# georgegrosu1/torch-admm-deconv

Hardware: AMD Instinct MI355X
Metric: ADMM iterations/sec, batch-64 1024x1024x3, 50 iters; rel-L2 vs CPU ref (higher is better)
Workload: dtype f32

## Files before the change

torch-admm-deconv_amd/csrc/admm_capi.hip:

```cpp
#include <hip/hip_runtime.h>

#include <cstdlib>
#include <cstring>
#include <mutex>
#include <string>
#include <type_traits>
#include <vector>

#include "gcol_mm.hpp"
#include "knobs.hpp"
#include "mixed_capi.hpp"
#include "odd_capi.hpp"
#include "admm_tv.h"

using namespace admm;

namespace {

thread_local std::string g_err;

int fail(int code, const std::string& msg) {
    g_err = msg;
    return code;
}
// ... 221 lines not shown
int launch_check(const char* what) {
    hipError_t e = hipGetLastError();
    if (e != hipSuccess) return fail(ADMM_TV_EHIP, std::string(what) + ": " + hipGetErrorString(e));
    return 0;
}

int hip_code(hipError_t e, const char* what) {
    return e == hipSuccess ? 0 : fail(ADMM_TV_EHIP, std::string(what) + ": " + hipGetErrorString(e));
}

int check_workspace(const void* ws, size_t have, size_t need) {
    if (!ws || have < need || (reinterpret_cast<uintptr_t>(ws) % kAlign) != 0)
        return fail(ADMM_TV_EWORKSPACE, "workspace too small or not 256-byte aligned");
    return 0;
}

template <class T>
int bwd_scalars(double* part, int K, long long nstrips, long long spm, long long soff, const double* tpart, int ntp,
                int G, int g, const T* lam, const T* rho, T* glam, T* grho, hipStream_t s) {
    if (K < 1) return fail(ADMM_TV_EINVAL, "bwd_scalars: no iterations");
    hipLaunchKernelGGL(k_bwd_iter_sums, dim3((unsigned)K), dim3(256), 0, s, part, nstrips, spm, soff, tpart, ntp, G, g);
    if (int e = launch_check("k_bwd_iter_sums")) return e;
    hipLaunchKernelGGL(k_bwd_scalars<T>, dim3(1), dim3(256), 0, s, (const double*)part, K, nstrips, 1LL, soff,
                       (const double*)nullptr, ntp, G, g, lam, rho, glam, grho);
    return launch_check("k_bwd_scalars");
}

template <int N> struct RowOps {
    using G = RowKernelGeom<N>;
    static unsigned blocks(long long items) { return (unsigned)((items + G::SG - 1) / G::SG); }

    static int r2c(const float* img, cf* spec, const cf* twW, long long rows, hipStream_t s, bool pl = false) {
        if (pl)
            hipLaunchKernelGGL((k_row_r2c<N, true>), dim3(blocks(rows)), dim3(G::NT), G::lds_bytes(), s, img, spec, twW, rows);
        else
            hipLaunchKernelGGL((k_row_r2c<N, false>), dim3(blocks(rows)), dim3(G::NT), G::lds_bytes(), s, img, spec, twW, rows);
        return launch_check("k_row_r2c");
    }
    static int c2r(const cf* spec, float* img, const cf* twW, long long rows, hipStream_t s, bool pl = false) {
        if (pl)
            hipLaunchKernelGGL((k_row_c2r<N, true>), dim3(blocks(rows)), dim3(G::NT), G::lds_bytes(), s, spec, img, twW, rows);
        else
            hipLaunchKernelGGL((k_row_c2r<N, false>), dim3(blocks(rows)), dim3(G::NT), G::lds_bytes(), s, spec, img, twW, rows);
        return launch_check("k_row_c2r");
    }
    static int pair(const float* img, float* out, long long rows, hipStream_t s) {
        hipLaunchKernelGGL(k_row_pair<N>, dim3(blocks(rows)), dim3(G::NT), 0, s, img, out, rows);
        return launch_check("k_row_pair");
    }
    template <bool ISO, bool FIRST, bool HIST, bool PL> static void pa(const PassAArgs& a, unsigned nb, hipStream_t s) {
        hipLaunchKernelGGL((k_pass_a<N, ISO, FIRST, HIST, PL>), dim3(nb), dim3(G::NT), G::lds_bytes(), s, a);
    }
    static constexpr bool kCoop = N == 512;
    template <bool FIRST, bool PL> static void pa_coop(const PassAArgs& a, unsigned nb, hipStream_t s) {
        if constexpr (kCoop)
            hipLaunchKernelGGL((k_pass_a<N, false, FIRST, false, PL, true>), dim3(nb), dim3(G::NT), passa_coop_lds<N>(), s, a);
    }
    static int pass_a(const PassAArgs& a, bool iso, bool first, bool hist, hipStream_t s, bool pl = false,
                      bool coop = false) {
        const unsigned nb = blocks(a.nstrips);
        const int sel = (iso ? 4 : 0) | (first ? 2 : 0) | (hist ? 1 : 0);
        if (kCoop && coop && !iso && !hist && !a.rev && a.R >= 2 && a.nstrips % G::SG == 0 &&
            (a.H / a.R) % G::SG == 0) {
            static_assert(!kCoop || passa_coop_lds<N>() <= 53 * 1024, "three blocks of the row pass per CU");
            if (first) pl ? pa_coop<true, true>(a, nb, s) : pa_coop<true, false>(a, nb, s);
            else pl ? pa_coop<false, true>(a, nb, s) : pa_coop<false, false>(a, nb, s);
            return launch_check("k_pass_a");
        }
        if (pl && !hist) {
            switch (sel) {
                case 0: pa<false, false, false, true>(a, nb, s); break;
                case 2: pa<false, true, false, true>(a, nb, s); break;
                case 4: pa<true, false, false, true>(a, nb, s); break;
                default: pa<true, true, false, true>(a, nb, s); break;
            }
            return launch_check("k_pass_a");
        }
        switch (sel) {
            case 0: pa<false, false, false, false>(a, nb, s); break;
            case 1: pa<false, false, true, false>(a, nb, s); break;
            case 2: pa<false, true, false, false>(a, nb, s); break;
            case 3: pa<false, true, true, false>(a, nb, s); break;
            case 4: pa<true, false, false, false>(a, nb, s); break;
            case 5: pa<true, false, true, false>(a, nb, s); break;
            case 6: pa<true, true, false, false>(a, nb, s); break;
            default: pa<true, true, true, false>(a, nb, s); break;
        }
        return launch_check("k_pass_a");
    }
    static int iso_norm(const IsoArgs& a, bool first, bool hist, hipStream_t s, bool pl = false) {
        const unsigned nb = blocks(a.nitems);
        if (first && pl)
            hipLaunchKernelGGL((k_iso_norm<N, true, false, true>), dim3(nb), dim3(G::NT), G::lds_bytes(), s, a);
        else if (first)
            hipLaunchKernelGGL((k_iso_norm<N, true, false, false>), dim3(nb), dim3(G::NT), G::lds_bytes(), s, a);
        else if (hist)
            hipLaunchKernelGGL((k_iso_norm<N, false, true, false>), dim3(nb), dim3(G::NT), G::lds_bytes(), s, a);
        else if (pl)
            hipLaunchKernelGGL((k_iso_norm<N, false, false, true>), dim3(nb), dim3(G::NT), G::lds_bytes(), s, a);
        else
            hipLaunchKernelGGL((k_iso_norm<N, false, false, false>), dim3(nb), dim3(G::NT), G::lds_bytes(), s, a);
        return launch_check("k_iso_norm");
    }
    template <bool ISO, bool LASTK, bool FIRSTK> static void bpa(const BwdArgs& a, unsigned nb, hipStream_t s) {
        using BG = BwdGeom<N>;
        hipLaunchKernelGGL((k_bwd_pass_a<N, ISO, LASTK, FIRSTK>), dim3(nb), dim3(BG::NT), BG::lds_bytes(), s, a);
    }
    static int bwd_pass_a(const BwdArgs& a, bool iso, bool lastk, bool firstk, hipStream_t s) {
        const unsigned nb = (unsigned)((a.nstrips + BwdGeom<N>::SG - 1) / BwdGeom<N>::SG);
        const int sel = (iso ? 4 : 0) | (lastk ? 2 : 0) | (firstk ? 1 : 0);
        switch (sel) {
            case 0: bpa<false, false, false>(a, nb, s); break;
            case 1: bpa<false, false, true>(a, nb, s); break;
            case 2: bpa<false, true, false>(a, nb, s); break;
            case 3: bpa<false, true, true>(a, nb, s); break;
            case 4: bpa<true, false, false>(a, nb, s); break;
            case 5: bpa<true, false, true>(a, nb, s); break;
            case 6: bpa<true, true, false>(a, nb, s); break;
            default: bpa<true, true, true>(a, nb, s); break;
// ... 170 lines not shown
    hipLaunchKernelGGL(k_tables<C>, dim3((std::max(H, W) + nt - 1) / nt), dim3(nt), 0, s, at<C>(ws, Lo.twW),
                       at<C>(ws, Lo.twH), at<double2>(ws, Lo.twHd), H, W);
    if (int e = launch_check("k_tables")) return e;
    if (Lo.gen && !std::is_same<T, double>::value) {
        for (int dim = 0; dim < 2; ++dim) {
            const GPlan pl = make_plan(dim == 0 ? W : H);
            if (pl.ntab == 0) continue;
            hipLaunchKernelGGL(k_blue_tables, dim3((3 * 1024 * 64 + nt - 1) / nt), dim3(nt), 0, s,
                               at<cf>(ws, dim == 0 ? Lo.twW : Lo.twH), pl);
            if (int e = launch_check("k_blue_tables")) return e;
        }
    }
    if (k > 0) {
        const int n = k * (N + 1);
        hipLaunchKernelGGL(k_psf_rows<T>, dim3((n + nt - 1) / nt), dim3(nt), 0, s, kern, at<double2>(ws, Lo.G), k, N, W);
        if (int e = launch_check("k_psf_rows")) return e;
    }
    const int n = (N + 1) * H;
    if (rho) {
        for (int g = 0; g < ngroups_of(d); ++g) {
            hipLaunchKernelGGL(k_spectra<T>, dim3((n + nt - 1) / nt), dim3(nt), 0, s, at<double2>(ws, Lo.G),
                               at<double2>(ws, Lo.twHd), rho + g, at<T>(ws, Lo.fcT) + (size_t)g * n, at<C>(ws, Lo.mT),
                               k, H, N, W, Lo.sigma ? at<double2>(ws, Lo.sigma) : nullptr,
                               (std::is_same<T, double>::value ? 1.0 / ((double)H * W) : spectra_scale(H, W)));
            if (int e = launch_check("k_spectra")) return e;
            if constexpr (std::is_same<T, float>::value) if (!Lo.gen) {
                float* fc = at<float>(ws, Lo.fcT) + (size_t)g * n;
                hipLaunchKernelGGL(k_fc_pack, dim3((n + nt - 1) / nt), dim3(nt), 0, s, fc,
                                   fc + (size_t)ngroups_of(d) * n, H, N, col_e(H));
                if (int e = launch_check("k_fc_pack")) return e;
            }
            if constexpr (std::is_same<T, float>::value) if (Lo.mixed) {
                if (int e = hip_code(admm_mixed::fc_mixed(at<float>(ws, Lo.fcT) + (size_t)g * n,
                                                          at<float>(ws, Lo.fcM) + (size_t)g * (2 * N + 1) * H, H, N, s),
                                     "k_fc_mixed"))
                    return e;
            }
            if constexpr (std::is_same<T, float>::value) if (Lo.gen && Lo.mm.ok && ngroups_of(d) == 1) {
                float* fc = at<float>(ws, Lo.fcT);
                hipLaunchKernelGGL(k_fc_transpose, dim3(std::min(4096, (n + nt - 1) / nt)), dim3(nt), 0, s, fc, fc + n, H,
                                   N + 1);
                if (int e = launch_check("k_fc_transpose")) return e;
            }
        }
        if constexpr (std::is_same<T, float>::value) if (Lo.mixed && k > 0) {
            if (int e = hip_code(admm_mixed::mt_mixed(at<cf>(ws, Lo.mT), at<cf>(ws, Lo.mM), H, N, s), "k_mt_mixed")) return e;
        }
    }
    return 0;
}

int pow2_floor(int v);

int strip_rows(int H, int N, long long rows, bool aniso_fwd = false) {
    int R = env_int("ADMM_PASSA_R", 0);
    if (R > 0) R = pow2_floor(std::max(2, std::min(R, H)));
    if (R <= 0) {
        const int L = std::min(64, N / (N >= 1024 ? 16 : N >= 64 ? 8 : N >= 16 ? 4 : 2));
        long long want = 3LL * 1024 * 64 / L;
        R = 8;
        if (aniso_fwd && N == 256) {
            R = 16;
            want /= 2;
        }
        while (R > 2 && rows / R < want) R /= 2;
    }
    if (R > H) R = H;
    return R;
}

struct DeviceGuard {
    int prev = -1, dev = -1;
    hipError_t err = hipSuccess;
    explicit DeviceGuard(hipStream_t s) {
        err = hipGetDevice(&prev);
        if (err != hipSuccess) return;
        dev = prev;
        if (s) {
            hipDevice_t d = 0;
            err = hipStreamGetDevice(s, &d);
            if (err != hipSuccess) return;
            dev = (int)d;
        }
        if (dev != prev) err = hipSetDevice(dev);
    }
    ~DeviceGuard() {
        if (prev >= 0 && dev != prev) (void)hipSetDevice(prev);
    }
    int check() const {
        return err == hipSuccess ? 0 : fail(ADMM_TV_EHIP, std::string("device of the stream: ") + hipGetErrorString(err));
    }
};

constexpr int kMaxAux = 3;
struct AuxEntry {
    hipStream_t caller = nullptr, aux[kMaxAux] = {};
};
constexpr int kAuxDev = 64, kAuxPerDev = 32;
struct AuxPool {
    std::mutex mu;
    AuxEntry e[kAuxDev][kAuxPerDev];
    int used[kAuxDev] = {}, next[kAuxDev] = {};
} g_aux;

hipStream_t aux_stream(hipStream_t s, int dev, int k = 0) {
    if (dev < 0 || dev >= kAuxDev || k < 0 || k >= kMaxAux) return nullptr;
    std::lock_guard<std::mutex> lk(g_aux.mu);
    AuxEntry* row = g_aux.e[dev];
    AuxEntry* slot = nullptr;
    for (int i = 0; i < g_aux.used[dev] && !slot; ++i)
        if (row[i].caller == s) slot = &row[i];
    if (!slot) {
        if (g_aux.used[dev] < kAuxPerDev) {
            slot = &row[g_aux.used[dev]++];
        } else {
            slot = &row[g_aux.next[dev]];
            g_aux.next[dev] = (g_aux.next[dev] + 1) % kAuxPerDev;
// ... 755 lines not shown
}

long long mixed_slots(int N) {
    static std::mutex mu;
    static std::vector<std::pair<std::pair<int, int>, long long>> cache;
    int dev = 0;
    if (hipGetDevice(&dev) != hipSuccess) return 512;
    std::lock_guard<std::mutex> lk(mu);
    for (const auto& c : cache)
        if (c.first.first == dev && c.first.second == N) return c.second;
    long long slots = 0;
    int cus = 0;
    if (hipDeviceGetAttribute(&cus, hipDeviceAttributeMultiprocessorCount, dev) == hipSuccess)
        slots = (long long)cus * std::max(1, admm_mixed::pass_a_blocks_per_cu(N));
    if (slots <= 0) return 512;
    cache.push_back({{dev, N}, slots});
    return slots;
}
int strip_rows_mixed(int H, long long rows, int N, long long slots = 0) {
    if (const int e = env_int("ADMM_MIXED_R", 0); e > 0 && H % e == 0) return e;
    const int sg = 256 / std::max(1, admm_mixed::row_lanes(N));
    if (slots <= 0) slots = mixed_slots(N);
    int best = 1;
    double best_t = 1e300;
    for (int R = 1; R <= 32 && R <= H; ++R) {
        if (H % R) continue;
        const long long strips = rows / R;
        const long long blocks = (strips + sg - 1) / sg;
        const double t = (double)((blocks + slots - 1) / slots) * (R + 1);
        if (t < best_t - 1e-9 || (t < best_t + 1e-9 && R > best)) {
            best_t = t;
            best = R;
        }
    }
    return best;
}

struct FusedOps {
    const admm_tv_desc& d;
    const Layout& Lo;
    void* const ws;
    const int H, N;
    cf *const twW, *const twH;
    FusedOps(const admm_tv_desc& d_, const Layout& L, void* w)
        : d(d_), Lo(L), ws(w), H((int)d_.H), N((int)d_.W / 2), twW(at<cf>(w, L.twW)), twH(at<cf>(w, L.twH)) {}
};

struct Pow2Ops : FusedOps {
    static constexpr bool kPsfGrad = true;
    float* const fcT;
    cf* const mT;
    const bool coop;
    const int rev;
    Pow2Ops(const admm_tv_desc& d_, const Layout& L, void* w)
        : FusedOps(d_, L, w), fcT(at<float>(w, L.fcT)), mT(at<cf>(w, L.mT)),
          coop(env_int("ADMM_PASSA_COOP", 1) != 0), rev(env_int("ADMM_PASSA_REV", 0)) {}
    int modules_per_pass(int G) const { return G; }
    bool lane_paired(bool train) const { return !train && env_int("ADMM_PL", (d.iso || d.W < 1024) ? 1 : 0) != 0; }
    int strip(long long rows, bool aniso_fwd) const { return strip_rows(H, N, rows, aniso_fwd); }
    int r2c(const float* img, cf* spec, long long rows, hipStream_t s, bool pl = false) const {
        return with_row(N, [&](auto ops) { return decltype(ops)::r2c(img, spec, twW, rows, s, pl); });
    }
    int c2r(const cf* spec, float* img, long long rows, hipStream_t s) const {
        return with_row(N, [&](auto ops) { return decltype(ops)::c2r(spec, img, twW, rows, s); });
    }
    int col(const cf* in, cf* out, long long np, long long ppm, int , hipStream_t s) const {
        return pass_b_oop(H, in, out, fcT, mT, twH, N, (int)np, 0, s, (int)ppm);
    }
    int xspec(const cf* U, const cf* V, cf* part, long long P, int ppg, bool , hipStream_t s) const {
        return ::xspec(H, U, V, part, twH, N, (int)P, ppg, s);
    }
    int iso_norm(const IsoArgs& a, bool first, bool hist, hipStream_t s, bool pl) const {
        return with_row(N, [&](auto ops) { return decltype(ops)::iso_norm(a, first, hist, s, pl); });
    }
    int pass_a(const PassAArgs& a, bool iso, bool first, bool hist, hipStream_t s, bool pl) const {
        return with_row(N, [&](auto ops) { return decltype(ops)::pass_a(a, iso, first, hist, s, pl, coop); });
    }
    int bwd_iso_q(const BwdIsoArgs& a, bool lastk, hipStream_t s) const {
        return with_row(N, [&](auto ops) { return decltype(ops)::bwd_iso_q(a, lastk, s); });
    }
    int bwd_pass_a(const BwdArgs& a, bool iso, bool lastk, bool firstk, hipStream_t s) const {
        return with_row(N, [&](auto ops) { return decltype(ops)::bwd_pass_a(a, iso, lastk, firstk, s); });
    }
    int make_b(const float* xin, float* bb, cf* spec, bool pl, hipStream_t s) const {
        if (d.kh > 0) return psf_transpose_into(d, Lo, ws, xin, bb, spec, 1, s, pl);
        return with_row(N, [&](auto ops) { return decltype(ops)::pair(xin, bb, d.B * d.C * H, s); });
    }
    int apply_ht_t(const float* bbar, float* gxin, cf* spec, hipStream_t s) const {
        return psf_transpose_into(d, Lo, ws, bbar, gxin, spec, 2, s);
    }
};

struct MixedOps : FusedOps {
    static constexpr bool kPsfGrad = true;
    const float* const fcM;
    static constexpr int rev = 0;
    MixedOps(const admm_tv_desc& d_, const Layout& L, void* w) : FusedOps(d_, L, w), fcM(at<float>(w, L.fcM)) {}
    int modules_per_pass(int) const { return 1; }
    bool lane_paired(bool) const { return false; }
    int strip(long long rows, bool) const { return strip_rows_mixed(H, rows, N); }
    int r2c(const float* img, cf* spec, long long rows, hipStream_t s, bool = false) const {
        return hip_code(admm_mixed::r2c(N, img, spec, twW, rows, s), "k_row_r2c_m");
    }
    int c2r(const cf* spec, float* img, long long rows, hipStream_t s) const {
        return hip_code(admm_mixed::c2r(N, spec, img, twW, rows, s), "k_row_c2r_m");
    }
    int col(const cf* in, cf* out, long long np, long long, int g0, hipStream_t s) const {
        return hip_code(admm_mixed::pass_b(H, in, out, fcM + (size_t)g0 * (2 * N + 1) * H, twH, N, np, s), "k_pass_b_m");
    }
    int xspec(const cf* U, const cf* V, cf* part, long long P, int ppg, bool weighted, hipStream_t s) const {
        return hip_code(admm_mixed::xspec(H, U, V, part, twH, N, P, ppg, weighted ? 0.25f : 1.f, s), "k_xspec_m");
    }
    int iso_norm(const IsoArgs& a, bool first, bool hist, hipStream_t s, bool) const {
        return hip_code(admm_mixed::iso_norm(N, a, first, hist, s), "k_iso_norm_m");
    }
    int pass_a(const PassAArgs& a, bool iso, bool first, bool hist, hipStream_t s, bool) const {
        return hip_code(admm_mixed::pass_a(N, a, iso, first, hist, s), "k_pass_a_m");
    }
    int bwd_iso_q(const BwdIsoArgs& a, bool lastk, hipStream_t s) const {
        return hip_code(admm_mixed::bwd_iso_q(N, a, lastk, s), "k_bwd_iso_q_m");
    }
    int bwd_pass_a(const BwdArgs& a, bool iso, bool lastk, bool firstk, hipStream_t s) const {
        return hip_code(admm_mixed::bwd_pass_a(N, a, iso, lastk, firstk, s), "k_bwd_pass_a_m");
    }
    int make_b(const float* xin, float* bb, cf* spec, bool, hipStream_t s) const {
        const long long P = d.B * d.C;
        if (env_int("ADMM_MIXED_BGEN", 0)) return gapply<float>(xin, bb, spec, Lo, ws, d, 1, s);
        if (int e = r2c(xin, spec, P * H, s)) return e;
        if (int e = hip_code(admm_mixed::pass_b_cm(H, spec, at<cf>(ws, Lo.mM), twH, N, P, s), "k_pass_b_m<cm>")) return e;
// ... 683 lines not shown
```

torch-admm-deconv_amd/csrc/admm_kernels.hpp:

```cpp
#pragma once
#include "fft_core.hpp"

namespace admm {

template <int N, class Cfg = RowCfg<N>> struct RowXf {
    static constexpr int E = Cfg::E;
    static constexpr int L = N / E;
    static constexpr int W = 2 * N;
    static_assert(L <= 64, "row transforms keep one row inside one wave");

    __device__ __forceinline__ static void partner(const cf (&v)[E], cf (&p)[E], int t) {
        const int src = (L - t) & (L - 1);
#pragma unroll
        for (int j = 0; j < E; ++j) {
            float a = __shfl(v[E - 1 - j].x, src, L);
            float b = __shfl(v[E - 1 - j].y, src, L);
            p[j] = (t == 0) ? v[(E - j) & (E - 1)] : mkc(a, b);
        }
    }

    __device__ __forceinline__ static void c2r(cf (&v)[E], const RowBuf& buf, const cf* __restrict__ tw, int t) {
        cf p[E];
        partner(v, p, t);
#pragma unroll
        for (int j = 0; j < E; ++j) {
            const int k = t + L * j;
            cf z;
            if (j == 0 && t == 0) {
                z = mkc(v[0].x + v[0].y, v[0].x - v[0].y);
            } else {
                cf pc = cconj(p[j]);
                cf e = cadd(v[j], pc);
                cf o = cmulc(csub(v[j], pc), tw[k]);
                z = mkc(e.x - o.y, e.y + o.x);
            }
            v[j] = z;
        }
        fft_e<N, L, E, +1, 0, 2>(v, buf, tw, t, typename Cfg::S{});
    }

    __device__ __forceinline__ static void r2c(cf (&v)[E], const RowBuf& buf, const cf* __restrict__ tw, int t) {
        fft_e<N, L, E, -1, 0, 2>(v, buf, tw, t, typename Cfg::S{});
        cf p[E];
        partner(v, p, t);
#pragma unroll
        for (int j = 0; j < E; ++j) {
            const int k = t + L * j;
            cf z;
            if (j == 0 && t == 0) {
                z = mkc(2.f * (v[0].x + v[0].y), 2.f * (v[0].x - v[0].y));
            } else {
                cf pc = cconj(p[j]);
                cf s = cadd(v[j], pc);
                cf d = cmul(csub(v[j], pc), tw[k]);
                z = mkc(s.x + d.y, s.y - d.x);
            }
            v[j] = z;
        }
    }
};

__device__ __forceinline__ float soft(float a, float tau) {
    float m = fabsf(a) - tau;
    m = (m < 0.f) ? 0.f : m;
    return copysignf(m, a);
}
__device__ __forceinline__ float block_factor(float sumsq, float tau) {
    float n = sqrtf(sumsq + 1e-15f);
    float f = 1.f - tau / (n + 1e-15f);
    return f < 0.f ? 0.f : f;
}
template <class T> __device__ __forceinline__ constexpr T eps15() {
    if constexpr (std::is_same<T, float>::value) return 1e-15f;
    else return 1e-15;
}
__device__ __forceinline__ double soft(double a, double tau) {
    double m = fabs(a) - tau;
    m = (m < 0.0) ? 0.0 : m;
    return copysign(m, a);
}
__device__ __forceinline__ double block_factor(double sumsq, double tau) {
    double n = sqrt(sumsq + 1e-15);
    double f = 1.0 - tau / (n + 1e-15);
    return f < 0.0 ? 0.0 : f;
}

template <class C = cf>
__global__ void k_tables(C* __restrict__ twW, C* __restrict__ twH, double2* __restrict__ twHd, int H, int W) {
    using T = re_t<C>;
    const int i = blockIdx.x * blockDim.x + threadIdx.x;
    if (i < W) {
        double s, c;
        sincospi(2.0 * i / W, &s, &c);
        twW[i] = mkx<T>((T)c, (T)-s);
    }
// ... 42 lines not shown
    if (sigma_out) sigma_out[i] = make_double2(sr, si);
    const double rho = (double)rho_p[0];
    const double sx = sinpi((double)kx / W), sy = sinpi((double)ky / H);
    const double lap = 4.0 * sx * sx + 4.0 * sy * sy;
    fcT[i] = (T)(scale / (sr * sr + si * si + rho * lap));
    if (k > 0) {
        const int c = k / 2;
        const long long ph = (long long)c * ky * W + (long long)c * kx * H;
        const long long HW = (long long)H * W;
        double s, co;
        sincospi(2.0 * (double)(ph % HW) / (double)HW, &s, &co);
        mT[i] = mkx<T>((T)((sr * co - si * s) * scale), (T)((sr * s + si * co) * scale));
    }
}

template <int N> struct RowKernelGeom {
    static constexpr int E = RowCfg<N>::E, L = N / E, W = 2 * N;
    static constexpr int NT = 256, SG = NT / L;
    static constexpr size_t lds_bytes() { return sizeof(cf) * (W + SG * RowBuf::slots(N)); }
};

__device__ __forceinline__ void load_tw(cf* dst, const cf* __restrict__ src, int n) {
    for (int i = threadIdx.x; i < n; i += blockDim.x) dst[i] = src[i];
}

typedef float f4v __attribute__((ext_vector_type(4)));
template <int E, int L, bool PL, bool NT> __device__ __forceinline__ void ld_row(const cf* row, int t, cf (&v)[E]) {
    if constexpr (PL) {
        static_assert(E % 2 == 0, "lane-paired rows need an even number of values per lane");
        const f4v* r4 = reinterpret_cast<const f4v*>(row);
#pragma unroll
        for (int j = 0; j < E / 2; ++j) {
            const f4v q = NT ? __builtin_nontemporal_load(&r4[t + L * j]) : r4[t + L * j];
            v[2 * j] = mkc(q.x, q.y);
            v[2 * j + 1] = mkc(q.z, q.w);
        }
    } else {
#pragma unroll
        for (int j = 0; j < E; ++j) v[j] = ld_pol<NT>(&row[t + L * j]);
    }
}
template <int E, int L, bool PL, bool NT> __device__ __forceinline__ void st_row(cf* row, int t, const cf (&v)[E]) {
    if constexpr (PL) {
        f4v* r4 = reinterpret_cast<f4v*>(row);
#pragma unroll
        for (int j = 0; j < E / 2; ++j) {
            const f4v q = {v[2 * j].x, v[2 * j].y, v[2 * j + 1].x, v[2 * j + 1].y};
            if constexpr (NT) __builtin_nontemporal_store(q, &r4[t + L * j]);
            else r4[t + L * j] = q;
        }
    } else {
#pragma unroll
        for (int j = 0; j < E; ++j) st_pol<NT>(&row[t + L * j], v[j]);
    }
}

template <int N, bool PL>
__global__ void __launch_bounds__(256) k_row_r2c(const float* __restrict__ img, cf* __restrict__ spec,
                                                 const cf* __restrict__ twW_g, long long rows) {
    using G = RowKernelGeom<N>;
    constexpr int E = G::E, L = G::L;
    extern __shared__ __attribute__((aligned(16))) unsigned char smem[];
    cf* tw = reinterpret_cast<cf*>(smem);
    load_tw(tw, twW_g, G::W);
    __syncthreads();
    const int sgl = threadIdx.x / L, t = threadIdx.x % L;
    const long long row = (long long)blockIdx.x * G::SG + sgl;
    if (row >= rows) return;
    RowBuf buf{tw + G::W + sgl * RowBuf::slots(N)};
    const cf* src = reinterpret_cast<const cf*>(img + row * G::W);
    cf v[E];
    ld_row<E, L, PL, false>(src, t, v);
    RowXf<N>::r2c(v, buf, tw, t);
    cf* dst = spec + row * N;
#pragma unroll
    for (int j = 0; j < E; ++j) dst[t + L * j] = v[j];
}

template <int N, bool PL>
__global__ void __launch_bounds__(256) k_row_c2r(const cf* __restrict__ spec, float* __restrict__ img,
                                                 const cf* __restrict__ twW_g, long long rows) {
    using G = RowKernelGeom<N>;
    constexpr int E = G::E, L = G::L;
    extern __shared__ __attribute__((aligned(16))) unsigned char smem[];
    cf* tw = reinterpret_cast<cf*>(smem);
    load_tw(tw, twW_g, G::W);
    __syncthreads();
    const int sgl = threadIdx.x / L, t = threadIdx.x % L;
    const long long row = (long long)blockIdx.x * G::SG + sgl;
    if (row >= rows) return;
    RowBuf buf{tw + G::W + sgl * RowBuf::slots(N)};
    const cf* src = spec + row * N;
    cf v[E];
#pragma unroll
    for (int j = 0; j < E; ++j) v[j] = src[t + L * j];
    RowXf<N>::c2r(v, buf, tw, t);
    cf* dst = reinterpret_cast<cf*>(img + row * G::W);
    st_row<E, L, PL, false>(dst, t, v);
}

template <int N>
__global__ void __launch_bounds__(256) k_row_pair(const float* __restrict__ img, float* __restrict__ out, long long rows) {
    using G = RowKernelGeom<N>;
    constexpr int E = G::E, L = G::L;
    const int sgl = threadIdx.x / L, t = threadIdx.x % L;
    const long long row = (long long)blockIdx.x * G::SG + sgl;
// ... 250 lines not shown
    fft<H, L, +1, 1, 1>(v1, buf, tw, t);
#pragma unroll
    for (int j = 0; j < E; ++j) bstore_f4(ro, voff, j * sstep, make_float4(v0[j].x, v0[j].y, v1[j].x, v1[j].y));
}

struct PassAArgs {
    const cf* sin;
    cf* sout;
    const float* b;
    const float* uxi;
    const float* uyi;
    float* uxo;
    float* uyo;
    const float* nsq;
    const float* nsq_prev;
    const float* lam;
    const float* rho;
    const cf* twW;
    int H;
    int R;
    long long nstrips;
    long long ppm;
    int rev = 0;
};

#ifndef PASSA_MINW_SMALL
#define PASSA_MINW_SMALL 3
#endif
#define PASSA_MINW(n) ((n) >= 1024 ? 1 : PASSA_MINW_SMALL)

template <bool ISO, class T> __device__ __forceinline__ T shrink_z(T a, T tau, T nsum) {
    if constexpr (ISO) return block_factor(nsum, tau) * a;
    else return soft(a, tau);
}

template <bool ISO, bool FIRST, bool HIST>
__device__ __forceinline__ cf prev_u(const cf* __restrict__ src, const cf* __restrict__ nsp, size_t idx, float tau) {
    if constexpr (FIRST) {
        return mkc(0.f, 0.f);
    } else {
        const cf v = lda<16>(&src[idx]);
        if constexpr (HIST) {
            const cf n = ISO ? nsp[idx] : mkc(0.f, 0.f);
            return mkc(v.x - shrink_z<ISO>(v.x, tau, n.x), v.y - shrink_z<ISO>(v.y, tau, n.y));
        } else {
            return v;
        }
    }
}

template <int N> constexpr size_t passa_coop_lds() {
    return RowKernelGeom<N>::lds_bytes() + sizeof(cf) * (RowKernelGeom<N>::SG - 1) * N;
}
template <int N, bool ISO, bool FIRST, bool HIST, bool PL, bool COOP = false>
__global__ void __launch_bounds__(256, PASSA_MINW(N)) k_pass_a(PassAArgs a) {
    static_assert(!(PL && HIST), "the training history keeps the pixel-order layout");
    using G = RowKernelGeom<N>;
    constexpr int E = G::E, L = G::L, W = G::W, SG = G::SG;
    static_assert(!COOP || (L == 64 && SG % 2 == 0 && !HIST && !ISO), "cooperative strips: whole waves in pairs, aniso inference");
    constexpr bool kSpecNT = (ADMM_NT & 2) != 0 || ((ADMM_NT & 32) != 0 && N >= 512);
    extern __shared__ __attribute__((aligned(16))) unsigned char smem[];
    cf* tw = reinterpret_cast<cf*>(smem);
    load_tw(tw, a.twW, W);
    __syncthreads();
    const int sgl = COOP ? __builtin_amdgcn_readfirstlane(threadIdx.x / L) : threadIdx.x / L, t = threadIdx.x % L;
#ifndef ADMM_PASSA_REMAP
#define ADMM_PASSA_REMAP -1
#endif
    constexpr bool kRemap = ADMM_PASSA_REMAP < 0 ? N <= 256 : ADMM_PASSA_REMAP != 0;
    const unsigned blk = kRemap ? xcd_remap(blockIdx.x, gridDim.x) : blockIdx.x;
    long long strip = (long long)blk * G::SG + sgl;
    if constexpr (!COOP) {
        if (strip >= a.nstrips) return;
        if (a.rev) strip = a.nstrips - 1 - strip;
    }
    const int H = a.H, R = a.R;
    const int spp = H / R;
    const long long p = strip / spp;
    const int i0 = (int)(strip % spp) * R;
    RowBuf buf{tw + W + sgl * RowBuf::slots(N)};
    const int mod = (int)(p / a.ppm);
    const float rho = a.rho[mod];
    const float tau = a.lam[mod] / rho;

    const cf* sp = a.sin + (size_t)p * H * N;
    cf* so = a.sout + (size_t)p * H * N;
    const size_t poff = (size_t)p * H * W;
    const cf* bimg = reinterpret_cast<const cf*>(a.b + (size_t)(p - (long long)mod * a.ppm) * H * W);
    const cf* uxi = reinterpret_cast<const cf*>(a.uxi + poff);
    const cf* uyi = reinterpret_cast<const cf*>(a.uyi + poff);
    const bool ust = HIST || a.uxo != nullptr;
    cf* uxo = ust ? reinterpret_cast<cf*>(a.uxo + poff) : nullptr;
    cf* uyo = ust ? reinterpret_cast<cf*>(a.uyo + poff) : nullptr;
    const size_t moff = (size_t)mod * 2 * H * W;
    const cf* nsx = reinterpret_cast<const cf*>(a.nsq + moff);
    const cf* nsy = reinterpret_cast<const cf*>(a.nsq + moff + (size_t)H * W);
    const cf* npx = reinterpret_cast<const cf*>(a.nsq_prev + moff);
    const cf* npy = reinterpret_cast<const cf*>(a.nsq_prev + moff + (size_t)H * W);

    auto xrow = [&](int g, cf (&x)[E]) __attribute__((always_inline)) {
#pragma unroll
        for (int j = 0; j < E; ++j) x[j] = ld_pol<kSpecNT>(&sp[(size_t)g * N + t + L * j]);
        RowXf<N>::c2r(x, buf, tw, t);
    };
    auto ydir = [&](int g, const cf (&xg)[E], const cf (&xup)[E], bool store, cf (&wyc)[E]) __attribute__((always_inline)) {
        const size_t ro = (size_t)g * N;
        {
            cf uy[E], fy[E];
            if constexpr (PL) {
                if constexpr (FIRST) {
#pragma unroll
                    for (int j = 0; j < E; ++j) uy[j] = mkc(0.f, 0.f);
// ... 79 lines not shown
                const float n0 = a0 - z0, n1 = a1 - z1;
                ux[j] = HIST ? mkc(a0, a1) : mkc(n0, n1);
                wxp[j] = mkc(z0 - n0, z1 - n1);
            }
            if (ust) {
                if constexpr (PL) {
                    st_row<E, L, true, (ADMM_NT & 1) != 0>(uxo + ro, t, ux);
                } else {
#pragma unroll
                    for (int j = 0; j < E; ++j) sta(&uxo[ro + t + L * j], ux[j]);
                }
            }
        }
    };

    cf xprev[E], xcur[E], wxp[E], wyp[E], wyc[E];
    auto pick = [](bool c, cf p, cf q) __attribute__((always_inline)) { return mkc(c ? p.x : q.x, c ? p.y : q.y); };
    auto ystep = [&](bool up, int gy, bool store) __attribute__((always_inline)) {
        cf xg[E], xup[E];
#pragma unroll
        for (int j = 0; j < E; ++j) {
            xg[j] = pick(up, xprev[j], xcur[j]);
            xup[j] = pick(up, xcur[j], xprev[j]);
        }
        ydir(gy, xg, xup, store, wyc);
    };
    auto fstep = [&](bool up, int gf) __attribute__((always_inline)) {
        cf wa[E], wb[E];
#pragma unroll
        for (int j = 0; j < E; ++j) {
            wa[j] = pick(up, wyc[j], wyp[j]);
            wb[j] = pick(up, wyp[j], wyc[j]);
        }
        finish(gf, wxp, wa, wb);
    };
    auto shift = [&]() __attribute__((always_inline)) {
#pragma unroll
        for (int j = 0; j < E; ++j) {
            wyp[j] = wyc[j];
            xprev[j] = xcur[j];
        }
    };
    auto step = [&](bool up, int g, bool ystore, bool fin, bool xd) __attribute__((always_inline)) {
        xrow(g, xcur);
        const int gn = up ? (g + 1) & (H - 1) : g;
        ystep(up, gn, ystore);
        if (fin) fstep(up, up ? gn : (g - 1 + H) & (H - 1));
        if (xd) xdir(g, xcur, wxp);
        shift();
    };
    if constexpr (!COOP) {
        xrow((i0 - 1 + H) & (H - 1), xprev);
        for (int rr = 0; rr <= R; ++rr) step(false, (i0 + rr) & (H - 1), rr < R, rr >= 1, rr < R);
    } else {
        cf* mbox = tw + W + SG * RowBuf::slots(N);
        const bool up = (sgl & 1) != 0, top = sgl == 0, bot = sgl == SG - 1;
        cf* mbs = mbox + (size_t)min(max(up ? sgl : sgl - 1, 0), SG - 2) * N;
        cf* mbe = mbox + (size_t)(up ? sgl - 1 : sgl) * N;
        auto put = [&](cf* mb, const cf (&v)[E]) __attribute__((always_inline)) {
#pragma unroll
            for (int j = 0; j < E; ++j) mb[t + L * j] = v[j];
        };
        auto get = [&](const cf* mb, cf (&v)[E]) __attribute__((always_inline)) {
#pragma unroll
            for (int j = 0; j < E; ++j) v[j] = mb[t + L * j];
        };
        const int gs = up ? i0 + R - 1 : i0;
        if (top || bot) xrow((top ? i0 - 1 + H : i0 + R) & (H - 1), xprev);
        xrow(gs, xcur);
        if (up && !bot) put(mbs, xcur);
        lds_barrier();
        if (!up && !top) get(mbs, xprev);
        if (!up || bot) ystep(up, up ? (i0 + R) & (H - 1) : gs, !up);
        if (!up && !top) put(mbs, wyc);
        lds_barrier();
        if (up && !bot) get(mbs, wyc);
        xdir(gs, xcur, wxp);
        shift();
        for (int rr = 1; rr < R; ++rr) step(up, up ? i0 + R - 1 - rr : i0 + rr, true, true, true);
        if (!up) put(mbe, xprev);
        lds_barrier();
        if (up) {
            get(mbe, xcur);
            ystep(true, i0, true);
            put(mbe, wyc);
        }
        lds_barrier();
        if (!up) get(mbe, wyc);
        fstep(up, up ? i0 : i0 + R - 1);
    }
}

struct IsoArgs {
    const cf* sin;
    const float* uxi;
    const float* uyi;
    const float* nsq_prev;
    const float* lam;
    const float* rho;
    float* partial;
    const cf* twW;
    int P, H, ppg;
    long long nitems;
    long long ppm;
};

// ... 96 lines not shown
```

torch-admm-deconv_amd/csrc/fft_core.hpp:

```cpp
#pragma once
#include <hip/hip_runtime.h>
#include <type_traits>

namespace admm {

typedef float2 cf;

__device__ __forceinline__ cf mkc(float r, float i) { cf z; z.x = r; z.y = i; return z; }
__device__ __forceinline__ cf cadd(cf a, cf b) { return mkc(a.x + b.x, a.y + b.y); }
__device__ __forceinline__ cf csub(cf a, cf b) { return mkc(a.x - b.x, a.y - b.y); }
__device__ __forceinline__ cf cmul(cf a, cf b) {
    return mkc(fmaf(a.x, b.x, -(a.y * b.y)), fmaf(a.x, b.y, a.y * b.x));
}
__device__ __forceinline__ cf cmulc(cf a, cf b) {
    return mkc(fmaf(a.x, b.x, a.y * b.y), fmaf(a.y, b.x, -(a.x * b.y)));
}
__device__ __forceinline__ cf cconj(cf a) { return mkc(a.x, -a.y); }
__device__ __forceinline__ cf cscale(cf a, float s) { return mkc(a.x * s, a.y * s); }
template <int DIR> __device__ __forceinline__ cf mul_i(cf a) {
    return DIR < 0 ? mkc(a.y, -a.x) : mkc(-a.y, a.x);
}

typedef double2 cd;
__device__ __forceinline__ cd mkcd(double r, double i) { cd z; z.x = r; z.y = i; return z; }
// ... 126 lines not shown
    __device__ __forceinline__ static void combine(cf (&v)[E], cf (&e)[R / 2], cf (&o)[R / 2]) {
        if constexpr (K < R / 2) {
            cf t = tw_mul<R, DIR, K>(o[K]);
            v[OFF + K * STRIDE] = cadd(e[K], t);
            v[OFF + (K + R / 2) * STRIDE] = csub(e[K], t);
            combine<K + 1, STRIDE, OFF>(v, e, o);
        }
    }
    template <int STRIDE, int OFF, int E> __device__ __forceinline__ static void run(cf (&v)[E]) {
        cf e[R / 2], o[R / 2];
#pragma unroll
        for (int i = 0; i < R / 2; ++i) {
            e[i] = v[OFF + (2 * i) * STRIDE];
            o[i] = v[OFF + (2 * i + 1) * STRIDE];
        }
        DFT<R / 2, DIR>::template run<1, 0>(e);
        DFT<R / 2, DIR>::template run<1, 0>(o);
        combine<0, STRIDE, OFF>(v, e, o);
    }
};

template <int... Rs> struct Sched {};

template <int N> struct RowCfg;
template <> struct RowCfg<8> { static constexpr int E = 2; using S = Sched<2, 2, 2>; };
template <> struct RowCfg<16> { static constexpr int E = 4; using S = Sched<4, 4>; };
template <> struct RowCfg<32> { static constexpr int E = 4; using S = Sched<4, 4, 2>; };
template <> struct RowCfg<64> { static constexpr int E = 8; using S = Sched<8, 8>; };
template <> struct RowCfg<128> { static constexpr int E = 8; using S = Sched<8, 8, 2>; };
template <> struct RowCfg<256> { static constexpr int E = 8; using S = Sched<8, 8, 4>; };
template <> struct RowCfg<512> { static constexpr int E = 8; using S = Sched<8, 8, 8>; };
template <> struct RowCfg<1024> { static constexpr int E = 16; using S = Sched<16, 16, 4>; };
template <> struct RowCfg<2048> { static constexpr int E = 16; using S = Sched<16, 16, 8>; };
template <> struct RowCfg<4096> { static constexpr int E = 16; using S = Sched<16, 16, 16>; };

struct RowBuf {
    cf* base;
    __device__ __forceinline__ cf& at(int i) const { return base[i + (i >> 3)]; }
    static constexpr int slots(int n) { return n + n / 8; }
};
template <int C> struct ColBuf {
    cf* base;
    __device__ __forceinline__ cf& at(int i) const { return base[i * C]; }
};

__device__ __forceinline__ void lds_barrier() {
    __builtin_amdgcn_fence(__ATOMIC_RELEASE, "workgroup", "local");
    __builtin_amdgcn_s_barrier();
    __builtin_amdgcn_fence(__ATOMIC_ACQUIRE, "workgroup", "local");
}
template <int SYNC> __device__ __forceinline__ void xsync() {
    if constexpr (SYNC == 2) {
        lds_barrier();
    } else if constexpr (SYNC) {
        __syncthreads();
    } else {
        __builtin_amdgcn_fence(__ATOMIC_RELEASE, "wavefront");
        __builtin_amdgcn_wave_barrier();
        __builtin_amdgcn_fence(__ATOMIC_ACQUIRE, "wavefront");
    }
}

template <int I, int NI, class F> __device__ __forceinline__ void static_for(F&& f) {
    if constexpr (I < NI) {
        f(std::integral_constant<int, I>{});
        static_for<I + 1, NI>(f);
    }
}

template <int N, int L, int E, int R, int NS, int DIR, bool FIRST, bool LAST, int SYNC, int TWMUL, class Buf>
__device__ __forceinline__ void stage(cf (&v)[E], const Buf& buf, const cf* __restrict__ tw, int t) {
    constexpr int Q = E / R;
    if constexpr (!FIRST) {
#pragma unroll
        for (int j = 0; j < E; ++j) v[j] = buf.at(t + L * j);
    }
    static_for<0, Q>([&](auto qc) {
        constexpr int q = decltype(qc)::value;
        if constexpr (NS > 1) {
            const int m = (t + L * q) & (NS - 1);
#pragma unroll
            for (int k = 1; k < R; ++k) {
                cf w = tw[(m * k) * (N / (NS * R)) * TWMUL];
                v[q + Q * k] = DIR < 0 ? cmul(v[q + Q * k], w) : cmulc(v[q + Q * k], w);
            }
        }
        DFT<R, DIR>::template run<Q, q>(v);
    });
    if constexpr (!LAST) {
        xsync<SYNC>();
#pragma unroll
        for (int q = 0; q < Q; ++q) {
            const int vt = t + L * q;
            const int base = (vt / NS) * NS * R + (vt & (NS - 1));
#pragma unroll
            for (int k = 0; k < R; ++k) buf.at(base + k * NS) = v[q + Q * k];
        }
        xsync<SYNC>();
    }
}

template <int N, int L, int E, int NS, int DIR, bool FIRST, int SYNC, int TWMUL, class Buf, int R, int... Rest>
__device__ __forceinline__ void run_sched(cf (&v)[E], const Buf& buf, const cf* __restrict__ tw, int t) {
    constexpr bool LAST = sizeof...(Rest) == 0;
    stage<N, L, E, R, NS, DIR, FIRST, LAST, SYNC, TWMUL>(v, buf, tw, t);
    if constexpr (!LAST) run_sched<N, L, E, NS * R, DIR, false, SYNC, TWMUL, Buf, Rest...>(v, buf, tw, t);
// ... 20 lines not shown
```

Measured before the change: 724.9.

## Software-pipeline next-row loads in cooperative pass-A walk using buffer loads

Adds a prefetching variant of the cooperative pass-A kernel for N=512 that issues buffer loads for the next row's x, u, and b data before computing on the current row. This overlaps global memory latency with the FFT and shrink work. It also adds a wavefront-scoped LDS-only sync mode for the row FFTs, sets strip rows to 4 for the cooperative aniso path, and lowers launch bounds to 2 waves to leave room for the extra prefetch registers. The trade-off is higher register pressure and lower occupancy. Out-of-range 'dead' loads are redirected past the buffer end so they return zero.

```diff
diff --git a/torch-admm-deconv_amd/csrc/admm_capi.hip b/torch-admm-deconv_amd/csrc/admm_capi.hip
--- a/torch-admm-deconv_amd/csrc/admm_capi.hip
+++ b/torch-admm-deconv_amd/csrc/admm_capi.hip
@@ -297,19 +297,24 @@
         hipLaunchKernelGGL((k_pass_a<N, ISO, FIRST, HIST, PL>), dim3(nb), dim3(G::NT), G::lds_bytes(), s, a);
     }
     static constexpr bool kCoop = N == 512;
-    template <bool FIRST, bool PL> static void pa_coop(const PassAArgs& a, unsigned nb, hipStream_t s) {
-        if constexpr (kCoop)
-            hipLaunchKernelGGL((k_pass_a<N, false, FIRST, false, PL, true>), dim3(nb), dim3(G::NT), passa_coop_lds<N>(), s, a);
+    template <bool FIRST, bool PL> static void pa_coop(const PassAArgs& a, unsigned nb, hipStream_t s, bool pf) {
+        if constexpr (kCoop) {
+            if (pf)
+                hipLaunchKernelGGL((k_pass_a<N, false, FIRST, false, PL, true, true>), dim3(nb), dim3(G::NT), passa_coop_lds<N>(), s, a);
+            else
+                hipLaunchKernelGGL((k_pass_a<N, false, FIRST, false, PL, true>), dim3(nb), dim3(G::NT), passa_coop_lds<N>(), s, a);
+        }
     }
     static int pass_a(const PassAArgs& a, bool iso, bool first, bool hist, hipStream_t s, bool pl = false,
-                      bool coop = false) {
+                      bool coop = false, bool pf = false) {
         const unsigned nb = blocks(a.nstrips);
         const int sel = (iso ? 4 : 0) | (first ? 2 : 0) | (hist ? 1 : 0);
         if (kCoop && coop && !iso && !hist && !a.rev && a.R >= 2 && a.nstrips % G::SG == 0 &&
             (a.H / a.R) % G::SG == 0) {
             static_assert(!kCoop || passa_coop_lds<N>() <= 53 * 1024, "three blocks of the row pass per CU");
-            if (first) pl ? pa_coop<true, true>(a, nb, s) : pa_coop<true, false>(a, nb, s);
-            else pl ? pa_coop<false, true>(a, nb, s) : pa_coop<false, false>(a, nb, s);
+            pf = pf && (long long)a.H * N * (long long)sizeof(cf) < (1LL << 31);
+            if (first) pl ? pa_coop<true, true>(a, nb, s, pf) : pa_coop<true, false>(a, nb, s, pf);
+            else pl ? pa_coop<false, true>(a, nb, s, pf) : pa_coop<false, false>(a, nb, s, pf);
             return launch_check("k_pass_a");
         }
         if (pl && !hist) {
@@ -586,7 +591,7 @@
 
 int pow2_floor(int v);
 
-int strip_rows(int H, int N, long long rows, bool aniso_fwd = false) {
+int strip_rows(int H, int N, long long rows, bool aniso_fwd = false, bool coop = false) {
     int R = env_int("ADMM_PASSA_R", 0);
     if (R > 0) R = pow2_floor(std::max(2, std::min(R, H)));
     if (R <= 0) {
@@ -597,6 +602,7 @@
             R = 16;
             want /= 2;
         }
+        if (coop && aniso_fwd && N == 512 && (H / 4) % 4 == 0) R = 4;
         while (R > 2 && rows / R < want) R /= 2;
     }
     if (R > H) R = H;
@@ -1458,12 +1464,14 @@
     cf* const mT;
     const bool coop;
     const int rev;
+    const bool pf;
     Pow2Ops(const admm_tv_desc& d_, const Layout& L, void* w)
         : FusedOps(d_, L, w), fcT(at<float>(w, L.fcT)), mT(at<cf>(w, L.mT)),
-          coop(env_int("ADMM_PASSA_COOP", 1) != 0), rev(env_int("ADMM_PASSA_REV", 0)) {}
+          coop(env_int("ADMM_PASSA_COOP", 1) != 0), rev(env_int("ADMM_PASSA_REV", 0)),
+          pf(env_int("ADMM_PASSA_PF", 1) != 0) {}
     int modules_per_pass(int G) const { return G; }
     bool lane_paired(bool train) const { return !train && env_int("ADMM_PL", (d.iso || d.W < 1024) ? 1 : 0) != 0; }
-    int strip(long long rows, bool aniso_fwd) const { return strip_rows(H, N, rows, aniso_fwd); }
+    int strip(long long rows, bool aniso_fwd) const { return strip_rows(H, N, rows, aniso_fwd, coop && !rev); }
     int r2c(const float* img, cf* spec, long long rows, hipStream_t s, bool pl = false) const {
         return with_row(N, [&](auto ops) { return decltype(ops)::r2c(img, spec, twW, rows, s, pl); });
     }
@@ -1480,7 +1488,7 @@
         return with_row(N, [&](auto ops) { return decltype(ops)::iso_norm(a, first, hist, s, pl); });
     }
     int pass_a(const PassAArgs& a, bool iso, bool first, bool hist, hipStream_t s, bool pl) const {
-        return with_row(N, [&](auto ops) { return decltype(ops)::pass_a(a, iso, first, hist, s, pl, coop); });
+        return with_row(N, [&](auto ops) { return decltype(ops)::pass_a(a, iso, first, hist, s, pl, coop, pf); });
     }
     int bwd_iso_q(const BwdIsoArgs& a, bool lastk, hipStream_t s) const {
         return with_row(N, [&](auto ops) { return decltype(ops)::bwd_iso_q(a, lastk, s); });
diff --git a/torch-admm-deconv_amd/csrc/admm_kernels.hpp b/torch-admm-deconv_amd/csrc/admm_kernels.hpp
--- a/torch-admm-deconv_amd/csrc/admm_kernels.hpp
+++ b/torch-admm-deconv_amd/csrc/admm_kernels.hpp
@@ -19,6 +19,7 @@
         }
     }
 
+    template <int SYNC = 0>
     __device__ __forceinline__ static void c2r(cf (&v)[E], const RowBuf& buf, const cf* __restrict__ tw, int t) {
         cf p[E];
         partner(v, p, t);
@@ -36,11 +37,12 @@
             }
             v[j] = z;
         }
-        fft_e<N, L, E, +1, 0, 2>(v, buf, tw, t, typename Cfg::S{});
-    }
-
+        fft_e<N, L, E, +1, SYNC, 2>(v, buf, tw, t, typename Cfg::S{});
+    }
+
+    template <int SYNC = 0>
     __device__ __forceinline__ static void r2c(cf (&v)[E], const RowBuf& buf, const cf* __restrict__ tw, int t) {
-        fft_e<N, L, E, -1, 0, 2>(v, buf, tw, t, typename Cfg::S{});
+        fft_e<N, L, E, -1, SYNC, 2>(v, buf, tw, t, typename Cfg::S{});
         cf p[E];
         partner(v, p, t);
 #pragma unroll
@@ -189,6 +191,34 @@
     } else {
 #pragma unroll
         for (int j = 0; j < E; ++j) st_pol<NT>(&row[t + L * j], v[j]);
+    }
+}
+
+template <int E, int L, bool PL, int AUX> __device__ __forceinline__ void bld_row(rsrc_t r, int voff, int soff, cf (&v)[E]) {
+    if constexpr (PL) {
+        static_assert(E % 2 == 0, "lane-paired rows need an even number of values per lane");
+#pragma unroll
+        for (int j = 0; j < E / 2; ++j) {
+            const f4v q = __builtin_bit_cast(f4v, __builtin_amdgcn_raw_buffer_load_b128(r, voff + L * j * 16, soff, AUX));
+            v[2 * j] = mkc(q.x, q.y);
+            v[2 * j + 1] = mkc(q.z, q.w);
+        }
+    } else {
+#pragma unroll
+        for (int j = 0; j < E; ++j) v[j] = bload_cf<AUX>(r, voff + L * j * 8, soff);
+    }
+}
+template <int E, int L, bool PL, int AUX> __device__ __forceinline__ void bst_row(rsrc_t r, int voff, int soff, const cf (&v)[E]) {
+    if constexpr (PL) {
+        typedef decltype(__builtin_amdgcn_raw_buffer_load_b128(r, 0, 0, 0)) V4;
+#pragma unroll
+        for (int j = 0; j < E / 2; ++j) {
+            const f4v q = {v[2 * j].x, v[2 * j].y, v[2 * j + 1].x, v[2 * j + 1].y};
+            __builtin_amdgcn_raw_buffer_store_b128(__builtin_bit_cast(V4, q), r, voff + L * j * 16, soff, AUX);
+        }
+    } else {
+#pragma unroll
+        for (int j = 0; j < E; ++j) bstore_cf<AUX>(r, voff + L * j * 8, soff, v[j]);
     }
 }
 
@@ -545,12 +575,13 @@
 template <int N> constexpr size_t passa_coop_lds() {
     return RowKernelGeom<N>::lds_bytes() + sizeof(cf) * (RowKernelGeom<N>::SG - 1) * N;
 }
-template <int N, bool ISO, bool FIRST, bool HIST, bool PL, bool COOP = false>
-__global__ void __launch_bounds__(256, PASSA_MINW(N)) k_pass_a(PassAArgs a) {
+template <int N, bool ISO, bool FIRST, bool HIST, bool PL, bool COOP = false, bool PF = false>
+__global__ void __launch_bounds__(256, PF ? 2 : PASSA_MINW(N)) k_pass_a(PassAArgs a) {
     static_assert(!(PL && HIST), "the training history keeps the pixel-order layout");
     using G = RowKernelGeom<N>;
     constexpr int E = G::E, L = G::L, W = G::W, SG = G::SG;
     static_assert(!COOP || (L == 64 && SG % 2 == 0 && !HIST && !ISO), "cooperative strips: whole waves in pairs, aniso inference");
+    static_assert(!PF || COOP, "the pipelined row step is built for the cooperative walk");
     constexpr bool kSpecNT = (ADMM_NT & 2) != 0 || ((ADMM_NT & 32) != 0 && N >= 512);
     extern __shared__ __attribute__((aligned(16))) unsigned char smem[];
     cf* tw = reinterpret_cast<cf*>(smem);
@@ -736,6 +767,152 @@
     if constexpr (!COOP) {
         xrow((i0 - 1 + H) & (H - 1), xprev);
         for (int rr = 0; rr <= R; ++rr) step(false, (i0 + rr) & (H - 1), rr < R, rr >= 1, rr < R);
+    } else if constexpr (PF) {
+        constexpr int kRowB = N * (int)sizeof(cf);
+        constexpr int kAuxS = kSpecNT ? 2 : 0, kAuxU = (ADMM_NT & 16) != 0 ? 2 : 0, kAuxW = (ADMM_NT & 1) != 0 ? 2 : 0;
+        const unsigned pB = (unsigned)H * (unsigned)kRowB;
+        const rsrc_t rsi = make_rsrc(sp, pB), rso = make_rsrc(so, pB), rbb = make_rsrc(bimg, pB);
+        const rsrc_t ruxi = make_rsrc(uxi, pB), ruyi = make_rsrc(uyi, pB);
+        const rsrc_t ruxo = make_rsrc(ust ? (void*)uxo : (void*)so, ust ? pB : 0u);
+        const rsrc_t ruyo = make_rsrc(ust ? (void*)uyo : (void*)so, ust ? pB : 0u);
+        const int v8 = t * 8, vu = t * (PL ? 16 : 8);
+        cf px[E], puy[E], pb[E], pux[E];
+        auto ldx = [&](int g, bool dead) __attribute__((always_inline)) {
+            bld_row<E, L, false, kAuxS>(rsi, v8 + (dead ? (int)pB : 0), g * kRowB, px);
+        };
+        auto lduy = [&](int g, bool dead) __attribute__((always_inline)) {
+            if constexpr (!FIRST) bld_row<E, L, PL, kAuxU>(ruyi, vu + (dead ? (int)pB : 0), g * kRowB, puy);
+        };
+        auto ldb = [&](int g) __attribute__((always_inline)) { bld_row<E, L, PL, kAuxU>(rbb, vu, g * kRowB, pb); };
+        auto ldux = [&](int g, bool dead) __attribute__((always_inline)) {
+            if constexpr (!FIRST) bld_row<E, L, PL, kAuxU>(ruxi, vu + (dead ? (int)pB : 0), g * kRowB, pux);
+        };
+        using More = std::true_type;
+        using Done = std::false_type;
+        auto pick = [](bool c, cf p, cf q) __attribute__((always_inline)) { return mkc(c ? p.x : q.x, c ? p.y : q.y); };
+        cf xprev[E], xcur[E], wxp[E], wyp[E], wyc[E];
+        auto xrowP = [&](cf (&x)[E], int gnext, bool dead) __attribute__((always_inline)) {
+#pragma unroll
+            for (int j = 0; j < E; ++j) x[j] = px[j];
+            ldx(gnext, dead);
+            RowXf<N>::template c2r<3>(x, buf, tw, t);
+        };
+        auto ydirP = [&](bool up, int gy, bool store, auto more, int gnext, bool dead) __attribute__((always_inline)) {
+            cf uy[E];
+#pragma unroll
+            for (int j = 0; j < E; ++j) {
+                const cf xg = pick(up, xprev[j], xcur[j]), xup = pick(up, xcur[j], xprev[j]);
+                const cf u0 = FIRST ? mkc(0.f, 0.f) : puy[j];
+                const float a0 = (xg.x - xup.x) + u0.x;
+                const float a1 = (xg.y - xup.y) + u0.y;
+                const float z0 = shrink_z<false>(a0, tau, 0.f);
+                const float z1 = shrink_z<false>(a1, tau, 0.f);
+                const float n0 = a0 - z0, n1 = a1 - z1;
+                uy[j] = mkc(n0, n1);
+                wyc[j] = mkc(z0 - n0, z1 - n1);
+            }
+            if constexpr (decltype(more)::value) lduy(gnext, dead);
+            bst_row<E, L, PL, kAuxW>(ruyo, vu + (store ? 0 : (int)pB), gy * kRowB, uy);
+        };
+        auto finishP = [&](bool up, int gm, auto more, int gnext) __attribute__((always_inline)) {
+            cf r[E], sh[E];
+#pragma unroll
+            for (int j = 0; j < E; ++j) sh[j].x = __shfl(wxp[j].x, (t + 1) & (L - 1), L);
+#pragma unroll
+            for (int j = 0; j < E; ++j) {
+                const cf wa = pick(up, wyc[j], wyp[j]), wb = pick(up, wyp[j], wyc[j]);
+                const float wr = (t == L - 1) ? sh[(j + 1) & (E - 1)].x : sh[j].x;
+                const float v0 = (wxp[j].x - wxp[j].y) + (wa.x - wb.x);
+                const float v1 = (wxp[j].y - wr) + (wa.y - wb.y);
+                r[j] = mkc(fmaf(rho, v0, pb[j].x), fmaf(rho, v1, pb[j].y));
+            }
+            if constexpr (decltype(more)::value) ldb(gnext);
+            RowXf<N>::template r2c<3>(r, buf, tw, t);
+#pragma unroll
+            for (int j = 0; j < E; ++j) bstore_cf<kAuxW>(rso, v8 + L * j * 8, gm * kRowB, r[j]);
+        };
+        auto xdirP = [&](int g, int gnext, bool dead) __attribute__((always_inline)) {
+            cf ux[E], sh[E];
+#pragma unroll
+            for (int j = 0; j < E; ++j) sh[j].x = __shfl(xcur[j].y, (t - 1) & (L - 1), L);
+#pragma unroll
+            for (int j = 0; j < E; ++j) {
+                const cf u0 = FIRST ? mkc(0.f, 0.f) : pux[j];
+                const float xl = (t == 0) ? sh[(j - 1) & (E - 1)].x : sh[j].x;
+                const float a0 = (xcur[j].x - xl) + u0.x;
+                const float a1 = (xcur[j].y - xcur[j].x) + u0.y;
+                const float z0 = shrink_z<false>(a0, tau, 0.f);
+                const float z1 = shrink_z<false>(a1, tau, 0.f);
+                const float n0 = a0 - z0, n1 = a1 - z1;
+                ux[j] = mkc(n0, n1);
+                wxp[j] = mkc(z0 - n0, z1 - n1);
+            }
+            ldux(gnext, dead);
+            bst_row<E, L, PL, kAuxW>(ruxo, vu, g * kRowB, ux);
+        };
+        auto shift = [&]() __attribute__((always_inline)) {
+#pragma unroll
+            for (int j = 0; j < E; ++j) {
+                wyp[j] = wyc[j];
+                xprev[j] = xcur[j];
+            }
+        };
+        cf* mbox = tw + W + SG * RowBuf::slots(N);
+        const bool up = (sgl & 1) != 0, top = sgl == 0, bot = sgl == SG - 1;
+        cf* mbs = mbox + (size_t)min(max(up ? sgl : sgl - 1, 0), SG - 2) * N;
+        cf* mbe = mbox + (size_t)(up ? sgl - 1 : sgl) * N;
+        auto put = [&](cf* mb, const cf (&v)[E]) __attribute__((always_inline)) {
+#pragma unroll
+            for (int j = 0; j < E; ++j) mb[t + L * j] = v[j];
+        };
+        auto get = [&](const cf* mb, cf (&v)[E]) __attribute__((always_inline)) {
+#pragma unroll
+            for (int j = 0; j < E; ++j) v[j] = mb[t + L * j];
+        };
+        const int gs = up ? i0 + R - 1 : i0;
+        const int g1 = up ? gs - 1 : gs + 1;
+        const int gbel = (i0 + R) & (H - 1);
+        ldx(top ? (i0 - 1 + H) & (H - 1) : bot ? gbel : gs, false);
+        lduy(bot ? gbel : gs, up && !bot);
+        ldb(gs);
+        ldux(gs, false);
+        if (top || bot) xrowP(xprev, gs, false);
+        xrowP(xcur, g1, false);
+        if (up && !bot) put(mbs, xcur);
+        lds_barrier();
+        if (!up && !top) get(mbs, xprev);
+        if (!up || bot) {
+            ydirP(up, up ? gbel : gs, !up, More{}, up ? gs : g1, false);
+        } else {
+            lduy(gs, false);
+            bst_row<E, L, PL, kAuxW>(ruyo, vu + (int)pB, 0, xcur);
+        }
+        if (!up && !top) put(mbs, wyc);
+        lds_barrier();
+        if (up && !bot) get(mbs, wyc);
+        xdirP(gs, g1, false);
+        shift();
+        for (int rr = 1; rr < R; ++rr) {
+            const int g = up ? i0 + R - 1 - rr : i0 + rr;
+            const bool last = rr == R - 1;
+            const int gx = (up ? g - 1 + H : g + 1) & (H - 1);
+            xrowP(xcur, gx, last);
+            const int gn = up ? g + 1 : g;
+            ydirP(up, gn, true, More{}, up ? g : gx, !up && last);
+            finishP(up, up ? gn : g - 1, More{}, g);
+            xdirP(g, gx, last);
+            shift();
+        }
+        if (!up) put(mbe, xprev);
+        lds_barrier();
+        if (up) {
+            get(mbe, xcur);
+            ydirP(true, i0, true, Done{}, 0, false);
+            put(mbe, wyc);
+        }
+        lds_barrier();
+        if (!up) get(mbe, wyc);
+        finishP(up, up ? i0 : i0 + R - 1, Done{}, 0);
     } else {
         cf* mbox = tw + W + SG * RowBuf::slots(N);
         const bool up = (sgl & 1) != 0, top = sgl == 0, bot = sgl == SG - 1;
diff --git a/torch-admm-deconv_amd/csrc/fft_core.hpp b/torch-admm-deconv_amd/csrc/fft_core.hpp
--- a/torch-admm-deconv_amd/csrc/fft_core.hpp
+++ b/torch-admm-deconv_amd/csrc/fft_core.hpp
@@ -202,6 +202,10 @@
 template <int SYNC> __device__ __forceinline__ void xsync() {
     if constexpr (SYNC == 2) {
         lds_barrier();
+    } else if constexpr (SYNC == 3) {
+        __builtin_amdgcn_fence(__ATOMIC_RELEASE, "wavefront", "local");
+        __builtin_amdgcn_wave_barrier();
+        __builtin_amdgcn_fence(__ATOMIC_ACQUIRE, "wavefront", "local");
     } else if constexpr (SYNC) {
         __syncthreads();
     } else {
```

After: 747.7 (median of 6 runs). 1.03x the previous value.
